# lwowlwowl/advanced_scrapper

Measured on AMD Instinct MI355X. Metric: article GB/s keyword-matched (S&P500 set) at 1 & 8 GPUs; % of HBM peak, higher is better.
Workload: dtype u8

## Files before the change

### advanced_scrapper_amd/csrc/kwmatch.hip

```cpp
#include <hip/hip_runtime.h>

#include <algorithm>
#include <cstdio>
#include <cstring>
#include <map>
#include <string>
#include <unordered_map>
#include <vector>

#include "kwmatch_kernels.hpp"
#include "kwmatch_fast_kernel.hpp"
#include "kwmatch_split.hpp"
#include "kwenv.hpp"

using namespace kw;

#ifndef RX_SPLIT_MAX_PAT
#define RX_SPLIT_MAX_PAT 16384
#endif

struct ScratchCaps {
    int nk = 0, nr = 0, ng = 0;
    int ns = 0;
    uint32_t item_cap = 0, out_cap = 0;
// ... 139 lines not shown
{
    uint32_t a = 2 * kfull_h(m);
    uint32_t b = m >= 1 ? (2 * m - 2) / 20 : 0;
    return a > b ? a : b;
}

struct QStats {
    std::unordered_map<uint32_t, uint32_t> c4;
    bool have = false;
    uint32_t count(const uint8_t *p) const
    {
        const uint32_t k = (uint32_t)p[0] | ((uint32_t)p[1] << 8) | ((uint32_t)p[2] << 16) | ((uint32_t)p[3] << 24);
        auto it = c4.find(k);
        uint32_t c = it == c4.end() ? 0u : it->second;
        const uint8_t b = p[0];
        const uint32_t h = (b >= 'a' && b <= 'z') ? 4u : (b == ' ' ? 2u : 0u);
        return have ? 4 * c + h : h;
    }
};

struct FastBuild {
    std::vector<uint32_t> s1, p2, l2, t3, b2, edge_pre, edge_suf;
    int has_short = 0;
    int has_t3 = 0;
    uint32_t gate[6] = {0, 0, 0, 0, 0, 0};
    std::vector<uint64_t> ht_key, as_head, sig, bsig;
    std::vector<uint32_t> ht_begin, ht_cnt, kl, as_len, as_use_begin, as_use_cnt, use_pat, use_info0, use_info1,
        rxk, boff;
    uint32_t ht_mask = 0;
    std::unordered_map<uint64_t, std::vector<uint32_t>> edge;
    std::vector<uint64_t> edge_key;
    std::vector<uint32_t> edge_begin, edge_cnt, edge_ent;
    uint32_t edge_mask = 0;
    std::vector<uint32_t> ht4, arec, urec, urec2;
    std::vector<int32_t> rxf_idx;
    std::vector<uint64_t> rxf_pm, rxf_any, rxf_ext_mask;
    std::vector<uint32_t> rxf_len, rxf_ext_off, rxf_ext_cp;
    std::vector<uint8_t> rx_bytes;
    std::vector<uint32_t> use_rxs, rxl;
    std::vector<uint64_t> use_wild;
};

struct RxShape {
    uint32_t npos = 0;
    uint32_t frames = 0;
    bool quant = false, at = false, wordb = false, alt = false, nopos = false;
    bool set_ext = false;
    bool lit_ext = false;
    bool fixed() const { return !quant && !at && !alt && !nopos && !set_ext && npos >= 1 && npos <= 64; }
};

bool rx_check(const int32_t *rows, int64_t b, int64_t e, RxShape &S, int64_t &minlen)
{
    auto unit = [&](int64_t &a, int64_t end, int64_t &mn) -> bool {
        const int32_t *t = rows + 4 * a;
        const int op = t[0] & 0xFF;
        if (t[0] & ~(0xFF | KW_RX_LAZY)) return false;
        if (op == KW_RX_AT) {
            if (t[0] != KW_RX_AT || t[1] < KW_AT_BOS || t[1] > KW_AT_NWORD || t[2] != 0 || t[3] != 0) return false;
            S.at = true;
            S.wordb |= t[1] == KW_AT_WORD || t[1] == KW_AT_NWORD;
            ++a;
            return true;
        }
        if (op != KW_RX_LIT && op != KW_RX_ANY && op != KW_RX_SET) return false;
        if (t[2] < 0 || (t[3] >= 0 && t[3] < t[2]) || t[3] < -1) return false;
        const bool rep = !(t[2] == 1 && t[3] == 1);
// ... 343 lines not shown
    B.ht_key.assign(hs, ~0ull);
    B.ht_begin.assign(hs, 0);
    B.ht_cnt.assign(hs, 0);
    for (auto &kv : keys) {
        uint32_t slot = fk_ht_slot(kv.first, B.ht_mask);
        while (B.ht_key[slot] != ~0ull) slot = (slot + 1) & B.ht_mask;
        B.ht_key[slot] = kv.first;
        B.ht_begin[slot] = (uint32_t)B.kl.size();
        B.ht_cnt[slot] = (uint32_t)kv.second.size();
        B.kl.insert(B.kl.end(), kv.second.begin(), kv.second.end());
    }
    if (B.kl.empty()) B.kl.push_back(0);
    B.ht4.assign((size_t)hs * 4, 0);
    for (uint32_t sl = 0; sl < hs; ++sl) {
        B.ht4[4 * sl] = (uint32_t)B.ht_key[sl];
        B.ht4[4 * sl + 1] = (uint32_t)(B.ht_key[sl] >> 32);
        B.ht4[4 * sl + 2] = B.ht_begin[sl];
        B.ht4[4 * sl + 3] = B.ht_cnt[sl];
    }
    for (uint32_t a : B.kl) {
        if (B.as_len.empty()) break;
        if (B.as_use_cnt[a] >= (1u << 24)) { err = "kw_compile: anchor with more than 2^24 uses"; return KW_EUNSUPPORTED; }
        B.arec.push_back((uint32_t)B.as_head[a]);
        B.arec.push_back((uint32_t)(B.as_head[a] >> 32));
        B.arec.push_back(B.as_use_begin[a]);
        B.arec.push_back((B.as_use_cnt[a] << 8) | B.as_len[a]);
    }
    const uint32_t rx_base = (uint32_t)(n_pat ? pat_off[n_pat] : 0) + 16;
    for (size_t u = 0; u < B.use_pat.size(); ++u) {
        const bool rxm = B.use_rxs[u] != 0xFFFFFFFFu;
        const uint32_t sb = rxm ? rx_base + B.use_rxs[u] : B.boff[B.use_pat[u]] + (B.use_info0[u] >> 16);
        const uint32_t sl = B.use_info1[u] & 0xFFFF;
        const uint8_t *sp = rxm ? B.rx_bytes.data() + B.use_rxs[u] : pat_bytes + sb;
        B.urec.push_back(B.use_info0[u]);
        B.urec.push_back(B.use_info1[u]);
        B.urec.push_back(B.use_pat[u]);
        B.urec.push_back(sb);
        uint64_t hd = 0, tl = 0;
        const uint32_t hl = sl < 8 ? sl : 8;
        for (uint32_t k = 0; k < hl; ++k) hd |= (uint64_t)sp[k] << (8 * k);
        for (uint32_t k = 0; k < hl; ++k) tl |= (uint64_t)sp[sl - hl + k] << (8 * k);
        B.urec2.push_back((uint32_t)hd);
        B.urec2.push_back((uint32_t)(hd >> 32));
        B.urec2.push_back((uint32_t)tl);
        B.urec2.push_back((uint32_t)(tl >> 32));
    }
    if (B.urec2.empty()) B.urec2.assign(4, 0);
    if (B.arec.empty()) B.arec.assign(4, 0);
    if (B.urec.empty()) B.urec.assign(4, 0);
    {
        uint32_t es = 256;
        while (es < 2 * B.edge.size()) es <<= 1;
        B.edge_mask = es - 1;
        B.edge_key.assign(es, 0);
        B.edge_begin.assign(es, 0);
        B.edge_cnt.assign(es, 0);
        for (auto &kv : B.edge) {
            uint32_t slot = (uint32_t)(kv.first >> 32) & B.edge_mask;
            while (B.edge_key[slot] != 0) slot = (slot + 1) & B.edge_mask;
            B.edge_key[slot] = kv.first;
            B.edge_begin[slot] = (uint32_t)B.edge_ent.size();
            B.edge_cnt[slot] = (uint32_t)kv.second.size();
            B.edge_ent.insert(B.edge_ent.end(), kv.second.begin(), kv.second.end());
        }
        if (B.edge_ent.empty()) B.edge_ent.push_back(0);
    }
    B.rxf_ext_off.push_back((uint32_t)B.rxf_ext_cp.size());
    if (B.rxf_len.empty()) { B.rxf_len.push_back(1); B.rxf_any.push_back(0); B.rxf_pm.resize(128, 0); }
    if (B.rxf_ext_cp.empty()) { B.rxf_ext_cp.push_back(0); B.rxf_ext_mask.push_back(0); }
    if (B.as_head.empty()) { B.as_head.push_back(0); B.as_len.push_back(0); B.as_use_begin.push_back(0); B.as_use_cnt.push_back(0); }
    if (B.use_pat.empty()) { B.use_pat.push_back(0); B.use_info0.push_back(0); B.use_info1.push_back(0); }
    if (B.use_wild.empty()) { B.use_wild.push_back(0); B.use_rxs.push_back(0xFFFFFFFFu); }
    return KW_OK;
}

bool is_word_h(const uint32_t *bits, uint32_t c)
{
    if (c >= 0x110000u) return false;
    return (bits[c >> 5] >> (c & 31)) & 1u;
}

template <class T>
// ... 330 lines not shown
            fclose(f);
        }
    }
    std::vector<uint8_t> all_bytes(pat_bytes, pat_bytes + (n_pat ? pat_off[n_pat] : 0));
    all_bytes.resize(all_bytes.size() + 16, 0);
    all_bytes.insert(all_bytes.end(), FB.rx_bytes.begin(), FB.rx_bytes.end());
    all_bytes.resize(all_bytes.size() + 16, 0);

    std::vector<uint8_t> blob;
    size_t o_filt = push_array(blob, filt), o_htk = push_array(blob, ht_key), o_htb = push_array(blob, ht_begin),
           o_htc = push_array(blob, ht_cnt), o_kl = push_array(blob, kl_anchor), o_ash = push_array(blob, as_head),
           o_aso = push_array(blob, as_off), o_asl = push_array(blob, as_len), o_asub = push_array(blob, as_use_begin),
           o_asuc = push_array(blob, as_use_cnt), o_asb = push_array(blob, as_bytes), o_up = push_array(blob, use_pat),
           o_ui = push_array(blob, use_info), o_pi = push_array(blob, pat_info), o_pco = push_array(blob, pat_cp_off),
           o_pc = push_array(blob, pat_cps), o_pma = push_array(blob, pm_ascii), o_peo = push_array(blob, pm_ext_off),
           o_pec = push_array(blob, pm_ext_cp), o_pem = push_array(blob, pm_ext_mask), o_rxo = push_array(blob, rxo),
           o_rxa = push_array(blob, atoms), o_wb = push_array(blob, wb), o_fc = push_array(blob, f_count_ge),
           o_sk = push_array(blob, sub_key), o_sb = push_array(blob, sub_begin), o_sc = push_array(blob, sub_cnt),
           o_sp = push_array(blob, sub_pat), o_rxm = push_array(blob, rx_mask);
    size_t f_s1 = push_array(blob, FB.s1), f_p2 = push_array(blob, FB.p2), f_b2 = push_array(blob, FB.b2), f_l2 = push_array(blob, FB.l2),
           f_t3 = push_array(blob, FB.t3), f_epre = push_array(blob, FB.edge_pre), f_esuf = push_array(blob, FB.edge_suf), f_htk = push_array(blob, FB.ht_key),
           f_htb = push_array(blob, FB.ht_begin), f_htc = push_array(blob, FB.ht_cnt), f_kl = push_array(blob, FB.kl),
           f_ash = push_array(blob, FB.as_head), f_asl = push_array(blob, FB.as_len),
           f_asub = push_array(blob, FB.as_use_begin), f_asuc = push_array(blob, FB.as_use_cnt),
           f_up = push_array(blob, FB.use_pat), f_ui0 = push_array(blob, FB.use_info0),
           f_ui1 = push_array(blob, FB.use_info1), f_rxk = push_array(blob, FB.rxk), f_boff = push_array(blob, FB.boff),
           f_pb = push_array(blob, all_bytes), f_sig = push_array(blob, FB.sig), f_bsig = push_array(blob, FB.bsig),
           f_ek = push_array(blob, FB.edge_key), f_eb = push_array(blob, FB.edge_begin),
           f_ec = push_array(blob, FB.edge_cnt), f_ee = push_array(blob, FB.edge_ent),
           f_rxi = push_array(blob, FB.rxf_idx), f_rxp = push_array(blob, FB.rxf_pm), f_rxa = push_array(blob, FB.rxf_any),
           f_rxl = push_array(blob, FB.rxf_len), f_rxeo = push_array(blob, FB.rxf_ext_off),
           f_rxec = push_array(blob, FB.rxf_ext_cp), f_rxem = push_array(blob, FB.rxf_ext_mask),
           f_ht4 = push_array(blob, FB.ht4), f_arec = push_array(blob, FB.arec), f_urec = push_array(blob, FB.urec),
           f_urec2 = push_array(blob, FB.urec2), f_tcps = push_array(blob, pat_tcps), f_txk = push_array(blob, tx_key),
           f_txv = push_array(blob, tx_val), f_txi = push_array(blob, tx_inv), f_tb = push_array(blob, pat_tbytes),
           f_uw = push_array(blob, FB.use_wild), f_prxl = push_array(blob, FB.rxl), f_txu = push_array(blob, txu_pat);

    HIPCHK(h, hipSetDevice(device));
    HIPCHK(h, hipMalloc(&h->d_tables, blob.size()));
    HIPCHK(h, hipMemcpy(h->d_tables, blob.data(), blob.size(), hipMemcpyHostToDevice));
    h->tables_bytes = blob.size();
    uint8_t *B = (uint8_t *)h->d_tables;
    DevTables &T = h->T;
    T.filt = (const uint32_t *)(B + o_filt);
    T.ht_key = (const uint32_t *)(B + o_htk);
    T.ht_begin = (const uint32_t *)(B + o_htb);
    T.ht_cnt = (const uint32_t *)(B + o_htc);
    T.ht_mask = ht_size - 1;
    T.ht_shift = 32 - ht_log;
    T.kl_anchor = (const uint32_t *)(B + o_kl);
    T.as_head = (const uint64_t *)(B + o_ash);
    T.as_off = (const uint32_t *)(B + o_aso);
    T.as_len = (const uint32_t *)(B + o_asl);
    T.as_use_begin = (const uint32_t *)(B + o_asub);
    T.as_use_cnt = (const uint32_t *)(B + o_asuc);
    T.as_bytes = (const uint8_t *)(B + o_asb);
    T.use_pat = (const uint32_t *)(B + o_up);
    T.use_info = (const uint32_t *)(B + o_ui);
    T.pat_info = (const uint32_t *)(B + o_pi);
    T.pat_cp_off = (const uint32_t *)(B + o_pco);
    T.pat_cps = (const uint32_t *)(B + o_pc);
    T.pm_ascii = (const uint64_t *)(B + o_pma);
    T.pm_ext_off = (const uint32_t *)(B + o_peo);
    T.pm_ext_cp = (const uint32_t *)(B + o_pec);
    T.pm_ext_mask = (const uint64_t *)(B + o_pem);
    T.rx_off = (const uint32_t *)(B + o_rxo);
    T.rx_atoms = (const int4 *)(B + o_rxa);
// ... 25 lines not shown
    F.ht_cnt = (const uint32_t *)(B + f_htc);
    F.ht_mask = FB.ht_mask;
    F.kl = (const uint32_t *)(B + f_kl);
    F.as_head = (const uint64_t *)(B + f_ash);
    F.as_len = (const uint32_t *)(B + f_asl);
    F.as_use_begin = (const uint32_t *)(B + f_asub);
    F.as_use_cnt = (const uint32_t *)(B + f_asuc);
    F.use_pat = (const uint32_t *)(B + f_up);
    F.use_info0 = (const uint32_t *)(B + f_ui0);
    F.use_info1 = (const uint32_t *)(B + f_ui1);
    F.pat_info = T.pat_info;
    F.pat_rxk = (const uint32_t *)(B + f_rxk);
    F.pat_boff = (const uint32_t *)(B + f_boff);
    F.pat_bytes = (const uint8_t *)(B + f_pb);
    F.pat_cp_off = T.pat_cp_off;
    F.pat_cps = T.pat_cps;
    F.pat_sig = (const uint64_t *)(B + f_sig);
    F.pat_bsig = (const uint64_t *)(B + f_bsig);
    F.f_count_ge = T.f_count_ge;
    F.sub_key = T.sub_key;
    F.sub_begin = T.sub_begin;
    F.sub_cnt = T.sub_cnt;
    F.sub_pat = T.sub_pat;
    F.sub_mask = T.sub_mask;
    F.edge_key = (const uint64_t *)(B + f_ek);
    F.edge_begin = (const uint32_t *)(B + f_eb);
    F.edge_cnt = (const uint32_t *)(B + f_ec);
    F.edge_ent = (const uint32_t *)(B + f_ee);
    F.edge_mask = FB.edge_mask;
    F.word_bits = T.word_bits;
    F.ht4 = (const uint4 *)(B + f_ht4);
    F.arec = (const uint4 *)(B + f_arec);
    F.urec = (const uint4 *)(B + f_urec);
    F.urec2 = (const uint4 *)(B + f_urec2);
    F.rxf_idx = (const int32_t *)(B + f_rxi);
    F.rxf_pm = (const uint64_t *)(B + f_rxp);
    F.rxf_any = (const uint64_t *)(B + f_rxa);
    F.rxf_len = (const uint32_t *)(B + f_rxl);
    F.rxf_ext_off = (const uint32_t *)(B + f_rxeo);
    F.rxf_ext_cp = (const uint32_t *)(B + f_rxec);
    F.rxf_ext_mask = (const uint64_t *)(B + f_rxem);
    F.f_first = f_first;
    F.empty_pat = empty_pat;
    F.pat_tcps = (const uint32_t *)(B + f_tcps);
    F.pat_tbytes = (const uint8_t *)(B + f_tb);
    F.tx_key = (const uint32_t *)(B + f_txk);
    F.tx_val = (const uint32_t *)(B + f_txv);
    F.tx_inv = (const uint32_t *)(B + f_txi);
    F.tx_unsafe_short = tx_unsafe_short;
    F.txu_pat = (const uint32_t *)(B + f_txu);
    F.n_txu = (uint32_t)txu_pat.size();
    F.use_wild = (const uint64_t *)(B + f_uw);
    F.pat_rxl = (const uint32_t *)(B + f_prxl);
    F.tx_unsafe_edge = tx_unsafe_edge;
    h->n_anchor_fast = (int)FB.as_len.size();

    hipDeviceProp_t prop;
    HIPCHK(h, hipGetDeviceProperties(&prop, device));
    h->cus = prop.multiProcessorCount;
    int bpc = 0;
    HIPCHK(h, hipOccupancyMaxActiveBlocksPerMultiprocessor(&bpc, (const void *)kw_scan_kernel, BLOCK, kScanLds));
    h->blocks_per_cu = bpc > 0 ? bpc : 1;
    bpc = 0;
    HIPCHK(h, hipOccupancyMaxActiveBlocksPerMultiprocessor(&bpc, (const void *)kw_resolve_kernel, RK_BLOCK, 0));
    h->resolve_blocks_per_cu = bpc > 0 ? bpc : 1;
    bpc = 0;
    HIPCHK(h, hipOccupancyMaxActiveBlocksPerMultiprocessor(&bpc, (const void *)kw_filter_kernel, FS_BLOCK, 0));
// ... 213 lines not shown
    {
        const uint64_t icap = std::min<uint64_t>(h->caps.item_cap, item_index_limit() / (uint64_t)n_regions);
        h->FS.item_cap = (uint32_t)icap;
        h->FS.item_grow = icap == h->caps.item_cap && !h->item_clamped ? 1u : 0u;
    }
    h->FS.bigq = EK_BIGQ;
    if (const char *e = kw_env("KW_TEST_BIGQ")) h->FS.bigq = (uint32_t)std::min(std::max(0, atoi(e)), EK_BIGQ);
    h->FS.dyn = dyn_groups ? 1 : 0;
    h->FS.chunk_groups = kchunk;
    const int nk = h->nk;
    HIPCHK(h, hipMemsetAsync(h->S.status, 0, 416, st));
    HIPCHK(h, hipMemsetAsync(h->out_cnt_all, 0, ((size_t)2 * nk + h->nr + h->ng) * 4, st));
    HIPCHK(h, hipMemsetAsync(h->FS.vcnt, 0, (size_t)nk * 20, st));
    HIPCHK(h, hipMemsetAsync(h->FS.dset, 0, (h->FS.dmask + 1) * 8, st));
    if (n_docs > 0) {
        HIPCHK(h, hipMemsetAsync(h->FS.ncnt, 0, (size_t)n_docs * 8, st));
        HIPCHK(h, hipMemsetAsync(h->FS.dflags, 0, (size_t)n_docs * 4, st));
    }
    HIPCHK(h, hipEventRecord(h->ev0, st));
    if (n_docs > 0)
        hipLaunchKernelGGL(kw_filter_kernel, dim3(nsb), dim3(FS_BLOCK), 0, st, h->FT, h->arena, h->doc_off, n_docs,
                           h->FS);
    HIPCHK(h, hipEventRecord(h->evf, st));
    static const int tx_bpc = kw_env("KW_TX_BLOCKS_PER_CU") ? std::max(1, atoi(kw_env("KW_TX_BLOCKS_PER_CU"))) : 8;
    HIPCHK(h, hipStreamWaitEvent(side, h->evf, 0));
    if (n_docs > 0)
        hipLaunchKernelGGL(kw_tx_kernel, dim3(std::max(1, (int)std::min<int64_t>((n_docs + TX_BLOCK - 1) / TX_BLOCK, (int64_t)h->cus * tx_bpc))),
                           dim3(TX_BLOCK), 0, side, h->FT, h->arena, h->doc_off, n_docs, h->FS);
    HIPCHK(h, hipEventRecord(h->evx, side));
    static const int probe_waves = kw_env("KW_PROBE_WAVES") ? std::max(1, atoi(kw_env("KW_PROBE_WAVES"))) : 0;
    if (n_docs > 0)
        hipLaunchKernelGGL(kw_probe_kernel, dim3((std::min(n_regions, probe_waves ? probe_waves : nsb * FS_WAVES) + PK_WAVES - 1) / PK_WAVES),
                           dim3(PK_BLOCK), 0, st, h->FT,
                           h->T, h->arena, h->doc_off, n_regions, h->FS);
    HIPCHK(h, hipEventRecord(h->evp, st));
    HIPCHK(h, hipStreamWaitEvent(st, h->evx, 0));
    if (n_docs > 0) {
        static const bool flat = !kw_env("KW_EPI_FLAT") || atoi(kw_env("KW_EPI_FLAT")) != 0;
        const bool txb = EF_TX_FLAT && (!kw_env("KW_TEST_EPI_TXB") || atoi(kw_env("KW_TEST_EPI_TXB")) != 0);
        if (flat && txb && h->FT.n_txu == 0)
            hipLaunchKernelGGL(kw_epi_flat_kernel<true>, dim3(neb), dim3(EK_BLOCK), 0, st, h->FT, h->arena,
                               h->doc_off, n_docs, h->FS, h->S);
        else if (flat)
            hipLaunchKernelGGL(kw_epi_flat_kernel<false>, dim3(neb), dim3(EK_BLOCK), 0, st, h->FT, h->arena,
                               h->doc_off, n_docs, h->FS, h->S);
        else
            hipLaunchKernelGGL(kw_epi_kernel, dim3(neb), dim3(EK_BLOCK), 0, st, h->FT, h->arena, h->doc_off, n_docs,
                               h->FS, h->S);
        HIPCHK(h, hipGetLastError());
    }
    h->ns = n_regions;
    HIPCHK(h, hipEventRecord(h->ev1, st));
    HIPCHK(h, hipStreamWaitEvent(side, h->ev1, 0));
    HIPCHK(h, hipEventRecord(h->evs0, side));
    if (n_docs > 0) {
        hipLaunchKernelGGL(kw_resolve_kernel, dim3(nrb), dim3(RK_BLOCK), 0, side, h->FT, h->T, h->arena, h->doc_off,
                           n_docs, h->FS, h->S);
        hipLaunchKernelGGL(kw_resolve_big_kernel, dim3(std::min(nrb * RK_WAVES, h->cus * 4)), dim3(WAVE), 0, side,
                           h->FT, h->T, h->arena, h->doc_off, h->FS, h->S);
        HIPCHK(h, hipGetLastError());
    }
    HIPCHK(h, hipEventRecord(h->evs1, side));
    if (n_docs > 0) {
        int G[4] = {1, 4, 4, 4};
        if (const char *e = kw_env("KW_TASK_G")) sscanf(e, "%d,%d,%d,%d", &G[0], &G[1], &G[2], &G[3]);
        auto task = [&](auto kern, int g, hipStream_t s) {
            g = std::max(1, std::min(g, 16));
// ... 360 lines not shown
```

### advanced_scrapper_amd/csrc/kwmatch_fast.hpp

```cpp
#pragma once
#include "kwmatch_device.hpp"

namespace kw {

constexpr int FK_S1_BITS = 19;
constexpr int FK_P2_WORDS = 2048;
#ifndef FK_L2_BITS_CFG
#define FK_L2_BITS_CFG 18
#endif
#ifndef FK_T3_BITS_CFG
#define FK_T3_BITS_CFG 16
#endif
#ifndef FK_B2_BITS_CFG
#define FK_B2_BITS_CFG 16
#endif
constexpr int FK_L2_BITS = FK_L2_BITS_CFG;
constexpr int FK_T3_BITS = FK_T3_BITS_CFG;
constexpr int FK_B2_BITS = FK_B2_BITS_CFG;
static_assert(FK_B2_BITS <= 16, "fk_b2h_index takes the high bits of a 16-bit index");
constexpr int FK_EDGE_BITS = 20;
constexpr int FK_ITEMS0 = 512;
constexpr int FK_ITEMS1 = 64;
constexpr int FK_ITEMS_MAX = FK_ITEMS0;
constexpr int FK_BIG0 = 4096;
constexpr int FK_BIG1 = 512;
constexpr int FK_CP_CAP = 16384;
constexpr int RK_WAVES = 4;
constexpr int RK_BLOCK = RK_WAVES * WAVE;
constexpr uint32_t FK_MUL1 = 0x9E3779u;
constexpr uint32_t FK_MUL2 = 0x85EBCA6Bu;
constexpr uint32_t FK_MUL3 = 0xC2B2AE35u;
constexpr uint32_t FK_MUL4 = 0x27D4EB2Fu;

constexpr int FK_S1_WORDS = 1 << (FK_S1_BITS - 5);
constexpr uint32_t FK_S1_M1 = 0xD2511Fu;
constexpr uint32_t FK_S1_M2 = 0x9E3779u;
constexpr uint32_t FK_S1_EXT_MAX = 16384;
constexpr int FK_L2_WORDS = 1 << (FK_L2_BITS - 5);
constexpr int FK_T3_WORDS = 1 << (FK_T3_BITS - 5);
constexpr int FK_B2_WORDS = 1 << (FK_B2_BITS - 5);
constexpr int FK_EDGE_WORDS = 1 << (FK_EDGE_BITS - 5);

enum FastUseKind : uint32_t { FU_UPPER = 0, FU_FULL = 1, FU_PIECE = 2, FU_EDGE = 3, FU_RXM = 3 };

enum RxKind : uint32_t { RXK_LITERAL = 0, RXK_REGEX = 1 };
constexpr uint32_t EDGE_MIN_M = 11, EDGE_MAX_M = 20;

constexpr uint32_t DH_N1_SHIFT = 10;
constexpr uint32_t DH_NEED = 1u << 17;
constexpr uint32_t DH_EDGE0 = 1u << 18;
constexpr uint32_t DH_EDGE1 = 1u << 19;
constexpr uint32_t DH_NA0 = 1u << 20;
constexpr uint32_t DH_NA1 = 1u << 21;
constexpr uint32_t DH_DEFER = 1u << 22;
constexpr uint32_t DH_TX = 1u << 23;
constexpr uint32_t DH_RESOLVE = 1u << 24;
static_assert(FK_ITEMS0 < 1024 && FK_ITEMS1 < 128, "item counts must fit the document header");

struct FastTables {
    const uint32_t *s1;
    const uint32_t *p2;
    const uint32_t *l2;
    const uint32_t *t3;
    const uint32_t *b2;
    const uint32_t *edge_pre;
    const uint32_t *edge_suf;
    int has_short;
    uint32_t gate[6];
    int has_t3;
    const uint64_t *ht_key;
    const uint32_t *ht_begin;
    const uint32_t *ht_cnt;
    uint32_t ht_mask;
    const uint32_t *kl;
    const uint64_t *as_head;
    const uint32_t *as_len;
    const uint32_t *as_use_begin;
    const uint32_t *as_use_cnt;
    const uint32_t *use_pat;
    const uint32_t *use_info0;
    const uint32_t *use_info1;
    const uint32_t *pat_info;
    const uint32_t *pat_rxk;
    const uint32_t *pat_boff;
    const uint8_t *pat_bytes;
    const uint32_t *pat_cp_off;
    const uint32_t *pat_cps;
    const uint64_t *pat_sig;
    const uint64_t *pat_bsig;
    const int32_t *f_count_ge;
    const uint64_t *sub_key;
    const uint32_t *sub_begin;
    const uint32_t *sub_cnt;
    const uint32_t *sub_pat;
    uint32_t sub_mask;
    const uint64_t *edge_key;
    const uint32_t *edge_begin;
    const uint32_t *edge_cnt;
    const uint32_t *edge_ent;
    uint32_t edge_mask;
    const uint32_t *word_bits;
    int f_first;
    int empty_pat;
    const uint4 *ht4;
    const uint4 *arec;
    const uint4 *urec;
    const uint4 *urec2;
    const int32_t *rxf_idx;
    const uint64_t *rxf_pm;
    const uint64_t *rxf_any;
    const uint32_t *rxf_len;
    const uint32_t *rxf_ext_off;
    const uint32_t *rxf_ext_cp;
    const uint64_t *rxf_ext_mask;
    const uint32_t *pat_tcps;
    const uint8_t *pat_tbytes;
    const uint32_t *tx_key;
    const uint32_t *tx_val;
    const uint32_t *tx_inv;
    int tx_unsafe_short;
    const uint32_t *txu_pat;
    uint32_t n_txu;
    int tx_unsafe_edge;
    const uint64_t *use_wild;
    const uint32_t *pat_rxl;
};

struct FastScratch {
    uint64_t *items;
    uint32_t item_cap;
    uint32_t bigq;
    uint32_t item_grow;
    uint2 *hdr;
    kw_hit *out;
    uint32_t *out_cnt;
    uint32_t out_cap;
    uint32_t *cps;
    uint32_t *cpbase;
    uint32_t *defer_list;
    uint32_t *defer_cnt;
// ... 78 lines not shown
```

### advanced_scrapper_amd/csrc/kwmatch_split.hpp

```cpp
#pragma once
#include "kwmatch_fast_kernel.hpp"

namespace kw {

#ifndef FS_WAVES_CFG
#define FS_WAVES_CFG 16
#endif
#ifndef FS_MINW
#define FS_MINW 1
#endif
#ifndef FS_EQ_TRIGGER
#define FS_EQ_TRIGGER 32
#endif
#ifndef FS_AHEAD
#define FS_AHEAD 3
#endif

constexpr int FS_WAVES = FS_WAVES_CFG;
constexpr int FS_BLOCK = FS_WAVES * WAVE;
constexpr int PK_WAVES = 4;
constexpr int PK_BLOCK = PK_WAVES * WAVE;
#ifndef PK_POOL_CFG
#define PK_POOL_CFG 768
#endif
// ... 390 lines not shown
        if (lane == 0) {
            S.ccnt[c] = ccur;
            if (ccur > S.cand_cap) {
                atomicOr(&S.status[0], ST_CAND_OVERFLOW);
                atomicMax(&S.cmax[0], ccur);
            }
        }
    }
    unsigned long long c1 = ncand;
#pragma unroll
    for (int dd = 32; dd >= 1; dd >>= 1) c1 += __shfl_xor(c1, dd, WAVE);
    if (lane == 0) {
        atomicAdd(&S.stats[0], c1);
        atomicAdd(&S.stats[8], (unsigned long long)ncand2);
    }
}

__device__ __forceinline__ bool rxm_match(const uint8_t *__restrict__ a, int64_t s0, const uint8_t *__restrict__ prog,
                                          uint32_t L, uint64_t wm)
{
    for (uint32_t k = 0; k < L; k += 8) {
        const uint64_t t = load8(a, s0 + k), p = load8(prog, k);
        const uint32_t nb = L - k < 8 ? L - k : 8;
        const uint64_t valid = nb >= 8 ? ~0ull : ((1ull << (8 * nb)) - 1);
        uint64_t wb = 0;
#pragma unroll
        for (int j = 0; j < 8; ++j) wb |= ((wm >> (k + j)) & 1ull) ? (0xFFull << (8 * j)) : 0ull;
        wb &= valid;
        if (((t ^ p) & valid & ~wb) != 0 || (zb64(t ^ 0x0A0A0A0A0A0A0A0Aull) & wb) != 0) return false;
    }
    return true;
}

__global__ __launch_bounds__(PK_BLOCK, PK_MINW) void kw_probe_kernel(FastTables FT, DevTables T, const uint8_t *__restrict__ arena,
                                                            const int64_t *__restrict__ off, int32_t n_regions,
                                                            FastScratch S)
{
    __shared__ uint64_t pool_all[PK_WAVES * PK_POOL];
    __shared__ uint8_t pown_all[PK_WAVES * PK_POOL];
    __shared__ uint32_t scnt_all[PK_WAVES * WAVE];
    const int lane = lane_id();
    const int wib = threadIdx.x / WAVE;
    uint64_t *pool = pool_all + wib * PK_POOL;
    uint8_t *pown = pown_all + wib * PK_POOL;
    uint32_t *scnt = scnt_all + wib * WAVE;
    uint32_t nanchor = 0;
    const int64_t n_waves = (int64_t)gridDim.x * PK_WAVES;
    for (int64_t region = S.dyn ? fk_next_group(S.gnext + 1, true, 0, 0) : (int64_t)blockIdx.x * PK_WAVES + wib;
         region < n_regions; region = fk_next_group(S.gnext + 1, S.dyn, region, n_waves)) {
    const uint32_t *cand = S.cand + (size_t)region * S.cand_cap;
    int32_t cur_group = -1;
    const uint32_t nc = min(S.ccnt[region], S.cand_cap);
    uint64_t *items = S.items + (size_t)region * S.item_cap;
    const uint32_t icap = S.item_cap;
    const uint32_t ibase = (uint32_t)((size_t)region * S.item_cap);
    uint32_t icur = 0;
    uint32_t last_doc = 0xFFFFFFFFu;
    scnt[lane] = 0;
    for (uint32_t c0 = 0; c0 < nc; c0 += WAVE) {
        const bool inb = c0 + (uint32_t)lane < nc;
        const uint32_t e = inb ? cand[c0 + lane] : 0u;
        const bool is_hdr = inb && (e & 7u) == 0u;
        int32_t grp = is_hdr ? (int32_t)(e >> 3) : -1;
#pragma unroll
        for (int d = 1; d < WAVE; d <<= 1) {
            const int32_t y = __shfl_up(grp, d, WAVE);
            if (lane >= d) grp = max(grp, y);
        }
        grp = max(grp, cur_group);
        cur_group = __shfl(grp, WAVE - 1, WAVE);
        const bool inr = inb && !is_hdr;
        const uint32_t doc = (uint32_t)grp * FG_DOCS + ((e >> 3) & (FG_DOCS - 1));
        const int64_t t0 = inr ? off[2 * (int64_t)doc] : 0;
        const int64_t t1 = inr ? off[2 * (int64_t)doc + 1] : 0;
        const int64_t t2 = inr ? off[2 * (int64_t)doc + 2] : 0;
        const bool valid = inr && t1 - t0 <= MAX_FIELD_BYTES && t2 - t1 <= MAX_FIELD_BYTES;
        const int32_t l1 = (int32_t)(t1 - t0), l2 = (int32_t)(t2 - t0);
        const int32_t pr = (int32_t)(e >> 8);
        const int f = pr < l1 ? 0 : 1;
        const int32_t fbr = f ? l1 : 0, fer = f ? l2 : l1;
        const int64_t p = t0 + pr;
        const uint64_t h8 = valid ? ld_u64_unaligned(arena, p) : 0ull;
        uint32_t rb[3], re[3];
        {
            uint4 hs[3];
            uint64_t key[3];
            uint32_t slot[3];
#pragma unroll
            for (int i = 0; i < 3; ++i) {
                const int Lk = 4 - i;
                const bool want = valid && ((e >> i) & 1u) && pr + Lk <= fer;
                key[i] = ((uint64_t)Lk << 32) | (h8 & ((1ull << (8 * Lk)) - 1));
                slot[i] = fk_ht_slot(key[i], FT.ht_mask);
                hs[i] = want ? FT.ht4[slot[i]] : make_uint4(~0u, ~0u, 0u, 0u);
            }
#pragma unroll
            for (int i = 0; i < 3; ++i) {
                rb[i] = re[i] = 0;
                for (;;) {
                    const uint64_t kk = (uint64_t)hs[i].x | ((uint64_t)hs[i].y << 32);
                    if (kk == key[i]) { rb[i] = hs[i].z; re[i] = hs[i].z + hs[i].w; break; }
                    if (kk == ~0ull) break;
                    slot[i] = (slot[i] + 1) & FT.ht_mask;
                    hs[i] = FT.ht4[slot[i]];
                }
            }
        }
        uint32_t tcur = rb[0], tend = re[0], b1 = rb[1], e1 = re[1], b2 = rb[2], e2 = re[2];
#if defined(PK_TIMING_SKIP) && PK_TIMING_SKIP == 2
        bool more = false;
        if (__ballot(valid && (tcur | b1 | b2) == 0xFFFFFFFFu)) nanchor += 1;
#else
        bool more = valid;
#endif
        uint32_t pn = 0;
// ... 22 lines not shown
                    }
                    continue;
                }
                if (b1 >= e1 && b2 >= e2) { more = false; break; }
                tcur = b1; tend = e1;
                b1 = b2; e1 = e2;
                b2 = e2 = 0;
            }
            if (more && tcur >= tend && b1 >= e1 && b2 >= e2) more = false;
            int total;
            const int ex = wave_excl_scan_dpp((int)(uc + uc1), &total);
#if defined(PK_TIMING_SKIP)
            total = 0;
#endif
            for (int g0 = 0; g0 < total; g0 += WAVE) {
                const int g = g0 + lane;
                bool pass = false;
                uint64_t item = 0;
                int owner = 0;
#pragma unroll
                for (int step = 32; step >= 1; step >>= 1) {
                    const int cnd = owner + step;
                    const int exc = __shfl(ex, cnd & 63, WAVE);
                    if (cnd < WAVE && exc <= g) owner = cnd;
                }
                const int exo = __shfl(ex, owner, WAVE);
                const uint32_t oub = (uint32_t)__shfl((int)ub, owner, WAVE);
                const uint32_t ouc = (uint32_t)__shfl((int)uc, owner, WAVE);
                const uint32_t oub1 = (uint32_t)__shfl((int)ub1, owner, WAVE);
                const uint32_t loc = (uint32_t)(g - exo);
                const uint32_t u = loc < ouc ? oub + loc : oub1 + (loc - ouc);
                const int32_t ppr = __shfl(pr, owner, WAVE);
                const int32_t ofbr = __shfl(fbr, owner, WAVE), ofer = __shfl(fer, owner, WAVE);
                const int64_t ot0 = rdlane64v(t0, owner);
                do {
                if (g >= total) break;
                const uint4 ur = FT.urec[u];
                const uint32_t kind = ur.x & 0xFF, aoff = (ur.x >> 8) & 0xFF;
                const uint32_t sblen = ur.y & 0xFFFF;
                const uint32_t pat = ur.z;
                const int32_t s0r = ppr - (int32_t)aoff;
                if (s0r < ofbr || s0r + (int32_t)sblen > ofer) break;
                const int64_t s0 = ot0 + s0r, fb = ot0 + ofbr, fe2 = ot0 + ofer;
                const uint4 u2 = FT.urec2[u];
                const uint64_t th = load8(arena, s0);
                const uint64_t tt = load8(arena, s0 + (sblen > 8 ? sblen - 8 : 0));
                const uint32_t pi = kind == FU_UPPER ? FT.pat_info[pat] : 0u;
                const bool hasp = kind == FU_UPPER && s0 > fb, hasn = kind == FU_UPPER && s0 + (int64_t)sblen < fe2;
                const uint32_t prevb = hasp ? (uint32_t)arena[s0 - 1] : 0u;
                const uint32_t nextb = hasn ? (uint32_t)arena[s0 + sblen] : 0u;
                const uint32_t hl = sblen < 8 ? sblen : 8;
                const uint64_t hm = hl >= 8 ? ~0ull : ((1ull << (8 * hl)) - 1);
                if (kind == FU_RXM) {
                    if (!rxm_match(arena, s0, FT.pat_bytes + ur.w, sblen, FT.use_wild[u])) break;
                } else {
                    if ((th ^ ((uint64_t)u2.x | ((uint64_t)u2.y << 32))) & hm) break;
                    if (sblen > 8 && tt != ((uint64_t)u2.z | ((uint64_t)u2.w << 32))) break;
                    if (sblen > 16 && !span_equal(arena, s0 + 8, FT.pat_bytes + ur.w + 8, sblen - 16)) break;
                }
                if (kind == FU_UPPER) {
                    const bool wf = (pi & PI_WORD_FIRST) != 0, wl = (pi & PI_WORD_LAST) != 0;
                    bool wp = false;
                    if (hasp) wp = is_word_cp(T, prevb < 0x80u ? prevb : decode_before(arena, fb, s0));
                    if (wp == wf) break;
                    bool wn = false;
                    if (hasn) {
                        uint32_t ch = nextb;
                        if (nextb >= 0x80u) decode_at(arena, s0 + sblen, fe2, &ch);
                        wn = is_word_cp(T, ch);
                    }
                    if (wn == wl) break;
                }
                item = ((uint64_t)pat << IT_PAT_SHIFT) | ((uint64_t)(uint32_t)(s0r - ofbr) << IT_POS_SHIFT) |
                       ((uint64_t)kind << IT_KIND_SHIFT) | (uint64_t)u;
                pass = true;
                } while (0);
                const uint64_t pm = __ballot(pass);
                if (pass) {
                    const uint32_t k = pn + (uint32_t)__builtin_popcountll(pm & ((1ull << lane) - 1));
                    if (k < (uint32_t)PK_POOL) { pool[k] = item; pown[k] = (uint8_t)owner; }
                    atomicAdd(&scnt[owner], 1u);
                }
                pn += (uint32_t)__builtin_popcountll(pm);
            }
            wave_sync();
        }
        const uint32_t nmine = scnt[lane];
        int itotal;
        const int iex = wave_excl_scan_dpp((int)nmine, &itotal);
        const bool ovf = pn > (uint32_t)PK_POOL || icur + (uint32_t)itotal > icap;
        const uint64_t withm = __ballot(nmine > 0);
        if (withm) {
            const uint64_t below = (1ull << lane) - 1;
            const uint64_t prevm = withm & below;
            const uint32_t pdoc = (uint32_t)__shfl((int)doc, prevm ? 63 - __builtin_clzll(prevm) : 0, WAVE);
            const uint32_t prev_doc = prevm ? pdoc : last_doc;
            if (nmine > 0) {
                if (doc != prev_doc) S.hdr[doc].x = ibase + icur + (uint32_t)iex;
                atomicAdd(f ? &S.ncnt[doc].y : &S.ncnt[doc].x, nmine);
                if (ovf) atomicOr(&S.dflags[doc], DH_DEFER);
            }
// ... 1031 lines not shown
```

Baseline: 588.0.

## Interleave use records, pack word flags, and stage per-group doc offsets in LDS

The two use-record tables are merged into one interleaved array, and the pattern's word-boundary flags are packed into spare bits of the pattern word, which removes a separate pat_info gather. The probe kernel now loads each doc group's offsets once per wave into shared memory and addresses the arena with 32-bit offsets from a per-wave base. Unaligned 8-byte reads use aligned dword loads combined with alignbyte. Documents whose span would overflow the 32-bit offset are flagged for deferral, which adds a fallback path and extra shared-memory use.

```diff
diff --git a/advanced_scrapper_amd/csrc/kwmatch.hip b/advanced_scrapper_amd/csrc/kwmatch.hip
--- a/advanced_scrapper_amd/csrc/kwmatch.hip
+++ b/advanced_scrapper_amd/csrc/kwmatch.hip
@@ -195,7 +195,7 @@
     std::vector<uint64_t> edge_key;
     std::vector<uint32_t> edge_begin, edge_cnt, edge_ent;
     uint32_t edge_mask = 0;
-    std::vector<uint32_t> ht4, arec, urec, urec2;
+    std::vector<uint32_t> ht4, arec, urec;
     std::vector<int32_t> rxf_idx;
     std::vector<uint64_t> rxf_pm, rxf_any, rxf_ext_mask;
     std::vector<uint32_t> rxf_len, rxf_ext_off, rxf_ext_cp;
@@ -605,22 +605,27 @@
         const uint32_t sb = rxm ? rx_base + B.use_rxs[u] : B.boff[B.use_pat[u]] + (B.use_info0[u] >> 16);
         const uint32_t sl = B.use_info1[u] & 0xFFFF;
         const uint8_t *sp = rxm ? B.rx_bytes.data() + B.use_rxs[u] : pat_bytes + sb;
+        uint32_t pw = B.use_pat[u];
+        if ((B.use_info0[u] & 0xFF) == FU_UPPER) {
+            const uint32_t pi = pat_info[B.use_pat[u]];
+            if (pi & PI_WORD_FIRST) pw |= UR_WORD_FIRST;
+            if (pi & PI_WORD_LAST) pw |= UR_WORD_LAST;
+        }
         B.urec.push_back(B.use_info0[u]);
         B.urec.push_back(B.use_info1[u]);
-        B.urec.push_back(B.use_pat[u]);
+        B.urec.push_back(pw);
         B.urec.push_back(sb);
         uint64_t hd = 0, tl = 0;
         const uint32_t hl = sl < 8 ? sl : 8;
         for (uint32_t k = 0; k < hl; ++k) hd |= (uint64_t)sp[k] << (8 * k);
         for (uint32_t k = 0; k < hl; ++k) tl |= (uint64_t)sp[sl - hl + k] << (8 * k);
-        B.urec2.push_back((uint32_t)hd);
-        B.urec2.push_back((uint32_t)(hd >> 32));
-        B.urec2.push_back((uint32_t)tl);
-        B.urec2.push_back((uint32_t)(tl >> 32));
-    }
-    if (B.urec2.empty()) B.urec2.assign(4, 0);
+        B.urec.push_back((uint32_t)hd);
+        B.urec.push_back((uint32_t)(hd >> 32));
+        B.urec.push_back((uint32_t)tl);
+        B.urec.push_back((uint32_t)(tl >> 32));
+    }
     if (B.arec.empty()) B.arec.assign(4, 0);
-    if (B.urec.empty()) B.urec.assign(4, 0);
+    if (B.urec.empty()) B.urec.assign(8, 0);
     {
         uint32_t es = 256;
         while (es < 2 * B.edge.size()) es <<= 1;
@@ -1017,7 +1022,7 @@
            f_rxl = push_array(blob, FB.rxf_len), f_rxeo = push_array(blob, FB.rxf_ext_off),
            f_rxec = push_array(blob, FB.rxf_ext_cp), f_rxem = push_array(blob, FB.rxf_ext_mask),
            f_ht4 = push_array(blob, FB.ht4), f_arec = push_array(blob, FB.arec), f_urec = push_array(blob, FB.urec),
-           f_urec2 = push_array(blob, FB.urec2), f_tcps = push_array(blob, pat_tcps), f_txk = push_array(blob, tx_key),
+           f_tcps = push_array(blob, pat_tcps), f_txk = push_array(blob, tx_key),
            f_txv = push_array(blob, tx_val), f_txi = push_array(blob, tx_inv), f_tb = push_array(blob, pat_tbytes),
            f_uw = push_array(blob, FB.use_wild), f_prxl = push_array(blob, FB.rxl), f_txu = push_array(blob, txu_pat);
 
@@ -1109,7 +1114,6 @@
     F.ht4 = (const uint4 *)(B + f_ht4);
     F.arec = (const uint4 *)(B + f_arec);
     F.urec = (const uint4 *)(B + f_urec);
-    F.urec2 = (const uint4 *)(B + f_urec2);
     F.rxf_idx = (const int32_t *)(B + f_rxi);
     F.rxf_pm = (const uint64_t *)(B + f_rxp);
     F.rxf_any = (const uint64_t *)(B + f_rxa);
@@ -1389,7 +1393,7 @@
     if (n_docs > 0)
         hipLaunchKernelGGL(kw_probe_kernel, dim3((std::min(n_regions, probe_waves ? probe_waves : nsb * FS_WAVES) + PK_WAVES - 1) / PK_WAVES),
                            dim3(PK_BLOCK), 0, st, h->FT,
-                           h->T, h->arena, h->doc_off, n_regions, h->FS);
+                           h->T, h->arena, h->doc_off, n_docs, n_regions, h->FS);
     HIPCHK(h, hipEventRecord(h->evp, st));
     HIPCHK(h, hipStreamWaitEvent(st, h->evx, 0));
     if (n_docs > 0) {
diff --git a/advanced_scrapper_amd/csrc/kwmatch_fast.hpp b/advanced_scrapper_amd/csrc/kwmatch_fast.hpp
--- a/advanced_scrapper_amd/csrc/kwmatch_fast.hpp
+++ b/advanced_scrapper_amd/csrc/kwmatch_fast.hpp
@@ -45,6 +45,9 @@
 
 enum RxKind : uint32_t { RXK_LITERAL = 0, RXK_REGEX = 1 };
 constexpr uint32_t EDGE_MIN_M = 11, EDGE_MAX_M = 20;
+constexpr uint32_t UR_PAT_MASK = (1u << 20) - 1;
+constexpr uint32_t UR_WORD_FIRST = 1u << 30, UR_WORD_LAST = 1u << 31;
+static_assert(64 - IT_PAT_SHIFT == 20, "the pattern word's spare bits lie above the item's pattern field");
 
 constexpr uint32_t DH_N1_SHIFT = 10;
 constexpr uint32_t DH_NEED = 1u << 17;
@@ -105,7 +108,6 @@
     const uint4 *ht4;
     const uint4 *arec;
     const uint4 *urec;
-    const uint4 *urec2;
     const int32_t *rxf_idx;
     const uint64_t *rxf_pm;
     const uint64_t *rxf_any;
diff --git a/advanced_scrapper_amd/csrc/kwmatch_split.hpp b/advanced_scrapper_amd/csrc/kwmatch_split.hpp
--- a/advanced_scrapper_amd/csrc/kwmatch_split.hpp
+++ b/advanced_scrapper_amd/csrc/kwmatch_split.hpp
@@ -446,18 +446,31 @@
     return true;
 }
 
+__device__ __forceinline__ uint64_t ld_u64_at(const uint8_t *__restrict__ a, uint32_t p)
+{
+    const uint32_t *w = (const uint32_t *)(a + (p & ~3u));
+    const uint32_t s = p & 3u;
+    const uint32_t x0 = w[0], x1 = w[1], x2 = w[2];
+    return (uint64_t)__builtin_amdgcn_alignbyte(x1, x0, s) | ((uint64_t)__builtin_amdgcn_alignbyte(x2, x1, s) << 32);
+}
+
 __global__ __launch_bounds__(PK_BLOCK, PK_MINW) void kw_probe_kernel(FastTables FT, DevTables T, const uint8_t *__restrict__ arena,
-                                                            const int64_t *__restrict__ off, int32_t n_regions,
-                                                            FastScratch S)
+                                                            const int64_t *__restrict__ off, int64_t n_docs,
+                                                            int32_t n_regions, FastScratch S)
 {
     __shared__ uint64_t pool_all[PK_WAVES * PK_POOL];
     __shared__ uint8_t pown_all[PK_WAVES * PK_POOL];
     __shared__ uint32_t scnt_all[PK_WAVES * WAVE];
+    __shared__ uint32_t gds_all[PK_WAVES * (FG_DOCS + 1)];
+    __shared__ uint32_t gdt_all[PK_WAVES * FG_DOCS];
     const int lane = lane_id();
-    const int wib = threadIdx.x / WAVE;
+    const int wib = __builtin_amdgcn_readfirstlane((int)(threadIdx.x / WAVE));
     uint64_t *pool = pool_all + wib * PK_POOL;
     uint8_t *pown = pown_all + wib * PK_POOL;
     uint32_t *scnt = scnt_all + wib * WAVE;
+    uint32_t *gds = gds_all + wib * (FG_DOCS + 1), *gdt = gdt_all + wib * FG_DOCS;
+    int32_t tab_group = -1;
+    int64_t tab_gb = 0, tab_len = 0;
     uint32_t nanchor = 0;
     const int64_t n_waves = (int64_t)gridDim.x * PK_WAVES;
     for (int64_t region = S.dyn ? fk_next_group(S.gnext + 1, true, 0, 0) : (int64_t)blockIdx.x * PK_WAVES + wib;
@@ -484,17 +497,47 @@
         grp = max(grp, cur_group);
         cur_group = __shfl(grp, WAVE - 1, WAVE);
         const bool inr = inb && !is_hdr;
-        const uint32_t doc = (uint32_t)grp * FG_DOCS + ((e >> 3) & (FG_DOCS - 1));
-        const int64_t t0 = inr ? off[2 * (int64_t)doc] : 0;
-        const int64_t t1 = inr ? off[2 * (int64_t)doc + 1] : 0;
-        const int64_t t2 = inr ? off[2 * (int64_t)doc + 2] : 0;
-        const bool valid = inr && t1 - t0 <= MAX_FIELD_BYTES && t2 - t1 <= MAX_FIELD_BYTES;
-        const int32_t l1 = (int32_t)(t1 - t0), l2 = (int32_t)(t2 - t0);
+        const uint32_t dk = (e >> 3) & (FG_DOCS - 1);
+        const uint32_t doc = (uint32_t)grp * FG_DOCS + dk;
+        uint32_t t0 = 0;
+        uint32_t l1 = 0, l2 = 0;
+        bool far = false;
+        int64_t bb = -1;
+        for (uint64_t todo = __ballot(inr); todo;) {
+            const int32_t g = __builtin_amdgcn_readlane(grp, __builtin_ctzll(todo));
+            if (g != tab_group) {
+                const int64_t d0 = (int64_t)g * FG_DOCS;
+                const int nd = (int)(n_docs - d0 < FG_DOCS ? n_docs - d0 : FG_DOCS);
+                const int64_t o0 = lane <= nd ? off[2 * (d0 + lane)] : 0;
+                const int64_t o1 = lane < nd ? off[2 * (d0 + lane) + 1] : 0;
+                tab_gb = rdlane64(o0, 0);
+                tab_len = rdlane64(o0, nd) - tab_gb;
+                wave_sync();
+                if (lane <= nd) gds[lane] = (uint32_t)(o0 - tab_gb);
+                if (lane < nd) gdt[lane] = (uint32_t)(o1 - tab_gb);
+                wave_sync();
+                tab_group = g;
+            }
+            if (bb < 0) bb = tab_gb & ~(int64_t)15;
+            const int64_t delta = tab_gb - bb;
+            const bool toofar = (uint64_t)(delta + tab_len) > 0xF0000000ull;
+            const bool mine = inr && grp == g;
+            if (mine) {
+                const uint32_t s = gds[dk];
+                t0 = (uint32_t)delta + s;
+                l1 = gdt[dk] - s;
+                l2 = gds[dk + 1] - s;
+                far = toofar;
+            }
+            todo &= ~__ballot(mine);
+        }
+        const uint8_t *__restrict__ ab = arena + (bb < 0 ? 0 : bb);
+        if (inr && far) atomicOr(&S.dflags[doc], DH_DEFER);
+        const bool valid = inr && !far && l1 <= (uint32_t)MAX_FIELD_BYTES && l2 - l1 <= (uint32_t)MAX_FIELD_BYTES;
         const int32_t pr = (int32_t)(e >> 8);
-        const int f = pr < l1 ? 0 : 1;
-        const int32_t fbr = f ? l1 : 0, fer = f ? l2 : l1;
-        const int64_t p = t0 + pr;
-        const uint64_t h8 = valid ? ld_u64_unaligned(arena, p) : 0ull;
+        const int f = pr < (int32_t)l1 ? 0 : 1;
+        const int32_t fbr = f ? (int32_t)l1 : 0, fer = f ? (int32_t)l2 : (int32_t)l1;
+        const uint64_t h8 = valid ? ld_u64_at(ab, t0 + (uint32_t)pr) : 0ull;
         uint32_t rb[3], re[3];
         {
             uint4 hs[3];
@@ -583,41 +626,40 @@
                 const uint32_t u = loc < ouc ? oub + loc : oub1 + (loc - ouc);
                 const int32_t ppr = __shfl(pr, owner, WAVE);
                 const int32_t ofbr = __shfl(fbr, owner, WAVE), ofer = __shfl(fer, owner, WAVE);
-                const int64_t ot0 = rdlane64v(t0, owner);
+                const uint32_t ot0 = (uint32_t)__shfl((int)t0, owner, WAVE);
                 do {
                 if (g >= total) break;
-                const uint4 ur = FT.urec[u];
+                const uint4 ur = FT.urec[2 * u];
                 const uint32_t kind = ur.x & 0xFF, aoff = (ur.x >> 8) & 0xFF;
                 const uint32_t sblen = ur.y & 0xFFFF;
-                const uint32_t pat = ur.z;
+                const uint32_t pat = ur.z & UR_PAT_MASK;
                 const int32_t s0r = ppr - (int32_t)aoff;
                 if (s0r < ofbr || s0r + (int32_t)sblen > ofer) break;
-                const int64_t s0 = ot0 + s0r, fb = ot0 + ofbr, fe2 = ot0 + ofer;
-                const uint4 u2 = FT.urec2[u];
-                const uint64_t th = load8(arena, s0);
-                const uint64_t tt = load8(arena, s0 + (sblen > 8 ? sblen - 8 : 0));
-                const uint32_t pi = kind == FU_UPPER ? FT.pat_info[pat] : 0u;
-                const bool hasp = kind == FU_UPPER && s0 > fb, hasn = kind == FU_UPPER && s0 + (int64_t)sblen < fe2;
-                const uint32_t prevb = hasp ? (uint32_t)arena[s0 - 1] : 0u;
-                const uint32_t nextb = hasn ? (uint32_t)arena[s0 + sblen] : 0u;
+                const uint32_t s0 = ot0 + (uint32_t)s0r, fb = ot0 + (uint32_t)ofbr, fe2 = ot0 + (uint32_t)ofer;
+                const uint4 u2 = FT.urec[2 * u + 1];
+                const uint64_t th = ld_u64_at(ab, s0);
+                const uint64_t tt = ld_u64_at(ab, s0 + (sblen > 8 ? sblen - 8 : 0));
+                const bool hasp = kind == FU_UPPER && s0 > fb, hasn = kind == FU_UPPER && s0 + sblen < fe2;
+                const uint32_t prevb = hasp ? (uint32_t)ab[s0 - 1] : 0u;
+                const uint32_t nextb = hasn ? (uint32_t)ab[s0 + sblen] : 0u;
                 const uint32_t hl = sblen < 8 ? sblen : 8;
                 const uint64_t hm = hl >= 8 ? ~0ull : ((1ull << (8 * hl)) - 1);
                 if (kind == FU_RXM) {
-                    if (!rxm_match(arena, s0, FT.pat_bytes + ur.w, sblen, FT.use_wild[u])) break;
+                    if (!rxm_match(ab, (int64_t)s0, FT.pat_bytes + ur.w, sblen, FT.use_wild[u])) break;
                 } else {
                     if ((th ^ ((uint64_t)u2.x | ((uint64_t)u2.y << 32))) & hm) break;
                     if (sblen > 8 && tt != ((uint64_t)u2.z | ((uint64_t)u2.w << 32))) break;
-                    if (sblen > 16 && !span_equal(arena, s0 + 8, FT.pat_bytes + ur.w + 8, sblen - 16)) break;
+                    if (sblen > 16 && !span_equal(ab, (int64_t)s0 + 8, FT.pat_bytes + ur.w + 8, sblen - 16)) break;
                 }
                 if (kind == FU_UPPER) {
-                    const bool wf = (pi & PI_WORD_FIRST) != 0, wl = (pi & PI_WORD_LAST) != 0;
+                    const bool wf = (ur.z & UR_WORD_FIRST) != 0, wl = (ur.z & UR_WORD_LAST) != 0;
                     bool wp = false;
-                    if (hasp) wp = is_word_cp(T, prevb < 0x80u ? prevb : decode_before(arena, fb, s0));
+                    if (hasp) wp = is_word_cp(T, prevb < 0x80u ? prevb : decode_before(ab, (int64_t)fb, (int64_t)s0));
                     if (wp == wf) break;
                     bool wn = false;
                     if (hasn) {
                         uint32_t ch = nextb;
-                        if (nextb >= 0x80u) decode_at(arena, s0 + sblen, fe2, &ch);
+                        if (nextb >= 0x80u) decode_at(ab, (int64_t)s0 + sblen, (int64_t)fe2, &ch);
                         wn = is_word_cp(T, ch);
                     }
                     if (wn == wl) break;
```

After: 590.9 (median of 6 runs). About the same (+0.5%).
